# google/sbsim

Measured on AMD Instinct MI355X. Metric: zone-updates/sec (env-steps/sec x 9 zones) at batch=64k buildings per GPU, higher is better.
Workload: dtype f64

## Files before the change

### sbsim_amd/csrc/sb_device.h

```cpp
#ifndef SBSIM_AMD_SB_DEVICE_H_
#define SBSIM_AMD_SB_DEVICE_H_

#include <hip/hip_runtime.h>

#include <stdint.h>

#include "sb_layout.h"
#include "sbsim_amd.h"

namespace sb {

constexpr double kCAir = 1006.0;
constexpr double kCWater = 4180.0;
constexpr double kRhoWater = 1000.0;
constexpr double kGravity = 9.8;
constexpr int kNScal = 20;
constexpr double kAgeNone = -1e300;
__host__ __device__ inline bool age_is_none(double age) { return age < -1e200; }
constexpr int kModeMask = 0xff, kValveBit = 0x100;

struct Dev {
  int B, H, W, Z, N, Np, ncls, pitch, NL;
  int S, nsteps;
  unsigned S_magic;
  int nbands, fast;
  int ts;
  int lds_wave_doubles;
  int off_agtab, off_zscr, off_zmode;
  const uint8_t *cls;
  const double *ctab;
  const int *czone;
  const int *zone_off;
  const int *zone_cells_l;
  const uint4 *zl16;
  const int *zblk_zone;
  int n_zblocks;
  const int4 *sched;
  const unsigned long long *smask;
  int reg;
  int NR;
  int P;
  int T;
  int state_doubles;
  const uint8_t *tcls;
  const uint8_t *tcset;
  const double *tmulS;
  int tmul_doubles;
  const double *csetab;
  int ncset;
  int csetab_doubles;
  int two_sym, two_level;
  double *two_abuf;
  const int *zs_off;
  int tail_set_base, tail_pad_set;
  int RS;
  int AS;
  int ZRS;
  int Ws;
  int stream_ms;
  int n_ring;
  double n_ring_f64;
  int lw[4], l0[2], rowbase[2], nch[2];
  int lag;
  int nslots;
  float pred_haste;
  float pred_slack;
  int two_skip;
  float skip_kappa;
  int pred_first;
  int lds_reg_bytes;
  int wg_per_cu;
  int r_seam, r_A, r_zscr, r_xchg, r_zoff, r_zmode;
  int r_cmap;
  const unsigned long long *cmapS;
  const unsigned long long *amapS;
  const unsigned long long *zmapS;
  const int *cell_state;
  double *ring;
  double *temp;
  double *zmean;
  double *zair;
  double *damper;
  double *qz;
  int *mode;
  double *scal;
  struct Bld *bld;
  double *gtabg;
  double *zsum;
  double *gsum;
  int *nsw;
  int *next_b;
  int sweep_wgs;
  int *redo_ctr;
  int *redo_list;
  double *redo_scratch;
  int redo_mode;
  int roll_exact;
  int dbg_redo_mod;
  int roll_free;
  int O, col_ahu, col_blr, col_aux;
  const int *col_zone;
  const double *obs_mean, *obs_sigma;
  int n_src, n_hist, hist_normalize;
  const int *src_dest, *hist_col, *hist_off;
  const double *hist_bins;
  const int *act_kind, *act_zone;
  const double *act_lo, *act_hi;
  const int *zone_act;
  int n_damper_actions;
  long long *dbg;
  int dbg_timeline;
  sb_params p;
  const double *bp;
  const double *ctab_b;
  int off_wtab;
};

__host__ __device__ __forceinline__ double param_field(const sb_params &p, int k) {
  switch (k) {
    case SB_BP_VAV_MAX_AIR_FLOW: return p.vav_max_air_flow;
    case SB_BP_VAV_MAX_WATER_FLOW: return p.vav_max_water_flow;
    case SB_BP_AHU_RECIRC: return p.ahu_recirc;
    case SB_BP_AHU_HEAT_SP: return p.ahu_heat_sp;
    case SB_BP_AHU_COOL_SP: return p.ahu_cool_sp;
    case SB_BP_AHU_DP: return p.ahu_dp;
    case SB_BP_AHU_EFF: return p.ahu_eff;
    case SB_BP_AHU_MAX_FLOW: return p.ahu_max_flow;
    case SB_BP_BLR_SETPOINT: return p.blr_setpoint;
    case SB_BP_BLR_HEAD: return p.blr_head;
    case SB_BP_BLR_PUMP_EFF: return p.blr_pump_eff;
    case SB_BP_BLR_HEATING_RATE: return p.blr_heating_rate;
    case SB_BP_BLR_COOLING_RATE: return p.blr_cooling_rate;
    case SB_BP_BLR_CONV: return p.blr_conv;
    case SB_BP_BLR_LEN: return p.blr_len;
    case SB_BP_BLR_RADIUS: return p.blr_radius;
    case SB_BP_BLR_CAPACITY: return p.blr_capacity;
    case SB_BP_BLR_INS_K: return p.blr_ins_k;
    case SB_BP_BLR_INS_THICK: return p.blr_ins_thick;
    case SB_BP_COMFORT_LO: return p.comfort_lo;
    case SB_BP_COMFORT_HI: return p.comfort_hi;
    case SB_BP_ECO_LO: return p.eco_lo;
    case SB_BP_ECO_HI: return p.eco_hi;
    case SB_BP_MAX_PROD: return p.max_prod;
    case SB_BP_MIN_PROD: return p.min_prod;
    case SB_BP_MAX_ELEC: return p.max_elec;
    case SB_BP_MAX_GAS: return p.max_gas;
    case SB_BP_PROD_DELTA: return p.prod_delta;
    case SB_BP_PROD_STIFF: return p.prod_stiff;
    case SB_BP_W_PROD: return p.w_prod;
    case SB_BP_W_COST: return p.w_cost;
    default: return p.w_carbon;
  }
}

__device__ __forceinline__ double bparam(const Dev &a, int k, int b) {
  return a.bp ? a.bp[(size_t)k * a.B + b] : param_field(a.p, k);
}

struct ClockView {
  const double *rows;
  const int *offs;
  int pos, prev, n_rows;
  int own_prev;
};

template <bool CLK>
__device__ __forceinline__ int clock_row(const ClockView &c, int b) {
  if constexpr (CLK) return c.offs[b] + c.pos;
  else return 0;
}
template <bool CLK>
__device__ __forceinline__ double clocked(const ClockView &c, int row, int field, double scalar) {
  if constexpr (CLK) return c.rows[(size_t)row * SB_CLOCK_FIELDS + field];
  else return scalar;
}

struct StepArgs {
  const float *actions;
  float *obs, *reward, *info;
  sb_step_in in;
  ClockView clk;
};

int launch_sweep_lds(const Dev &d, int workgroups, int waves_per_wg, size_t lds_bytes, hipStream_t stream);
int prepare_sweep_lds(const Dev &d, size_t lds_bytes);
int launch_sweep_reg(const Dev &d, int cus, hipStream_t stream);
int prepare_sweep_reg(const Dev &d);
int launch_sweep_roll(const Dev &d, hipStream_t stream);
int prepare_sweep_roll(const Dev &d);
int launch_sweep_two(const Dev &d, hipStream_t stream);
int prepare_sweep_two(const Dev &d);
int launch_sweep_band(const Dev &d, hipStream_t stream);
int prepare_sweep_band(const Dev &d);
int launch_sweep_stream(const Dev &d, double *abuf, int waves, hipStream_t stream);
int prepare_sweep_stream(const Dev &d, int waves);
int launch_sweep_stream_ms(const Dev &d, double *abuf, double *ebuf, int waves, hipStream_t stream);
int prepare_sweep_stream_ms(const Dev &d, int waves);

template <int CTRL, int ROW_MASK>
__device__ __forceinline__ double dpp_or_zero(double x) {
  const int lo = __builtin_amdgcn_update_dpp(0, __double2loint(x), CTRL, ROW_MASK, 0xf, true);
  const int hi = __builtin_amdgcn_update_dpp(0, __double2hiint(x), CTRL, ROW_MASK, 0xf, true);
  return __hiloint2double(hi, lo);
}
__device__ __forceinline__ double wave_sum(double v) {
  double t = v + dpp_or_zero<0x111, 0xf>(v);
  t += dpp_or_zero<0x112, 0xf>(v);
  t += dpp_or_zero<0x113, 0xf>(v);
  t += dpp_or_zero<0x114, 0xf>(t);
  t += dpp_or_zero<0x118, 0xf>(t);
  t += dpp_or_zero<0x142, 0xa>(t);
  t += dpp_or_zero<0x143, 0xc>(t);
  const int lo = __builtin_amdgcn_readlane(__double2loint(t), 63);
  const int hi = __builtin_amdgcn_readlane(__double2hiint(t), 63);
  return __hiloint2double(hi, lo);
}
__device__ __forceinline__ double wave_max(double v) {
  double t = fmax(v, dpp_or_zero<0x111, 0xf>(v));
  t = fmax(t, dpp_or_zero<0x112, 0xf>(v));
  t = fmax(t, dpp_or_zero<0x113, 0xf>(v));
  t = fmax(t, dpp_or_zero<0x114, 0xf>(t));
  t = fmax(t, dpp_or_zero<0x118, 0xf>(t));
  t = fmax(t, dpp_or_zero<0x142, 0xa>(t));
  t = fmax(t, dpp_or_zero<0x143, 0xc>(t));
  const int lo = __builtin_amdgcn_readlane(__double2loint(t), 63);
  const int hi = __builtin_amdgcn_readlane(__double2hiint(t), 63);
  return __hiloint2double(hi, lo);
}
__device__ __forceinline__ int wave_max_i32(int v) {
  int t = max(v, __builtin_amdgcn_update_dpp(0, v, 0x111, 0xf, 0xf, true));
  t = max(t, __builtin_amdgcn_update_dpp(0, v, 0x112, 0xf, 0xf, true));
  t = max(t, __builtin_amdgcn_update_dpp(0, v, 0x113, 0xf, 0xf, true));
  t = max(t, __builtin_amdgcn_update_dpp(0, t, 0x114, 0xf, 0xf, true));
  t = max(t, __builtin_amdgcn_update_dpp(0, t, 0x118, 0xf, 0xf, true));
  t = max(t, __builtin_amdgcn_update_dpp(t, t, 0x142, 0xa, 0xf, false));
  t = max(t, __builtin_amdgcn_update_dpp(t, t, 0x143, 0xc, 0xf, false));
  return __builtin_amdgcn_readlane(t, 63);
}
__device__ __forceinline__ double wave_min(double v) {
#pragma unroll
  for (int o = 32; o > 0; o >>= 1) v = fmin(v, __shfl_xor(v, o, 64));
  return v;
}

__device__ __forceinline__ double ahu_supply(double mixed, double heat_sp, double cool_sp) {
  if (mixed > cool_sp) return cool_sp;
  if (mixed < heat_sp) return heat_sp;
  return mixed;
}

__device__ __forceinline__ int default_control(int mode, double tz, double hsp, double csp) {
// ... 451 lines not shown
```

### sbsim_amd/csrc/sbsim_hip.hip

```cpp
#include <hip/hip_runtime.h>

#include <algorithm>
#include <cmath>
#include <cstdlib>
#include <cstring>
#include <memory>
#include <string>
#include <vector>

#include "sb_host.h"
#include "step_two_cfg.h"

#ifndef SB_EXPERIMENTAL
namespace sb {
int launch_sweep_stream_ms(const Dev &, double *, double *, int, hipStream_t) { return (int)hipErrorNotSupported; }
int prepare_sweep_stream_ms(const Dev &, int) { return (int)hipErrorNotSupported; }
}
#endif

using namespace sb;

namespace {

struct Knobs {
  PlanKnobs plan;
  bool force_jacobi_global = env_flag("SBSIM_FORCE_JACOBI_GLOBAL");
  int jacobi_global_wgs = std::max(0, env_int("SBSIM_DEBUG_JACOBI_GLOBAL_WGS", 0));
  bool two_no_skip = env_flag("SBSIM_TWO_NO_SKIP");
  float pred_haste = (float)env_double("SBSIM_DEBUG_PRED_HASTE", 1.0);
  float pred_slack = (float)env_double("SBSIM_DEBUG_PRED_SLACK", 1.0);
  int pred_first = getenv("SBSIM_DEBUG_PRED_FIRST") ? std::max(1, env_int("SBSIM_DEBUG_PRED_FIRST", 1)) : 0;
  float skip_kappa = (float)std::min(100.0, std::max(0.0, env_double("SBSIM_DEBUG_SKIP_KAPPA", 0.9)));
  bool roll_exact = env_int("SBSIM_ROLL_EXACT", 0) != 0;
  int force_redo = std::max(0, env_int("SBSIM_DEBUG_FORCE_REDO", 0));
  bool roll_free = env_int("SBSIM_ROLL_FREE", 1) != 0;
  bool force_generic = env_flag("SBSIM_FORCE_GENERIC_SWEEP");
  bool phase_timing = getenv("SBSIM_PHASE_TIMING") != nullptr;
  bool debug_timeline = getenv("SBSIM_DEBUG_TIMELINE") != nullptr;
};

struct ActionTable {
  std::vector<int> zone_act;
  int n_damper_actions = 0;
};

int check_create_args(const sb_plan_desc *plan, const sb_params *params, const sb_obs_layout *obs, int n_buildings,
                      ActionTable &acts) {
  int rc = check_plan(plan);
  if (rc != SB_OK) return rc;
  if (n_buildings < 1) return fail(SB_ERR_INVALID, "sb_create: n_buildings must be >= 1");
  if (params->dt <= 0 || params->iter_limit < 1)
    return fail(SB_ERR_INVALID, "sb_create: time_step_sec and iteration_limit must be positive");
  if (params->ahu_cool_sp <= params->ahu_heat_sp)
    return fail(SB_ERR_INVALID, "cooling_air_temp_setpoint must greater than heating_air_temp_setpoint");
  if (params->n_actions < 1 || params->n_actions > 3 + plan->Z)
    return fail(SB_ERR_INVALID, "sb_create: n_actions must be in 1 .. 3 + zones (one column per settable field)");
  if (!params->act_kind || !params->act_zone || !params->act_lo || !params->act_hi)
    return fail(SB_ERR_INVALID, "sb_create: null action table (sb_params.act_kind / act_zone / act_lo / act_hi)");
  acts.zone_act.assign((size_t)std::max(plan->Z, 1), -1);
  int seen[3] = {0, 0, 0};
  for (int i = 0; i < params->n_actions; ++i) {
    const int kind = params->act_kind[i];
    if (kind < SB_ACT_BOILER_SUPPLY_WATER_SETPOINT || kind > SB_ACT_VAV_SUPPLY_AIR_DAMPER_COMMAND)
      return fail(SB_ERR_INVALID, "sb_create: unknown action kind");
    if (kind == SB_ACT_VAV_SUPPLY_AIR_DAMPER_COMMAND) {
      const int z = params->act_zone[i];
      if (z < 0 || z >= plan->Z) return fail(SB_ERR_INVALID, "sb_create: VAV action for a zone the floor plan does not have");
      if (acts.zone_act[z] >= 0) return fail(SB_ERR_INVALID, "sb_create: two action columns drive the same VAV damper");
      acts.zone_act[z] = i;
      ++acts.n_damper_actions;
    } else if (seen[kind]++) {
      return fail(SB_ERR_INVALID, "sb_create: two action columns drive the same setpoint");
    }
  }
  if (obs->n_obs < 1) return fail(SB_ERR_INVALID, "sb_create: empty observation layout");
  if (!obs->mean || !obs->sigma || (plan->Z > 0 && !obs->col_zone))
    return fail(SB_ERR_INVALID, "sb_create: null observation-layout table");
  {
    const int n_fields = obs->n_src ? obs->n_src : obs->n_obs, n_ahu = params->ahu_has_weather ? 9 : 8;
    bool ok = obs->col_ahu >= 0 && obs->col_ahu + n_ahu <= n_fields && obs->col_boiler >= 0 &&
              obs->col_boiler + 3 <= n_fields && obs->col_aux >= 0 && obs->col_aux + SB_NUM_AUX <= obs->n_obs;
    for (int z = 0; z < plan->Z; ++z) ok = ok && obs->col_zone[z] >= 0 && obs->col_zone[z] + 3 <= n_fields;
    if (!ok) return fail(SB_ERR_INVALID, "sb_create: observation columns outside the observation row");
  }
  for (int z = 0; z < plan->Z; ++z)
    if (plan->zone_off[z + 1] == plan->zone_off[z]) return fail(SB_ERR_INVALID, "sb_create: a zone without cells");
  if (obs->n_src) {
    const int n_dev_fields = 3 * plan->Z + (params->ahu_has_weather ? 9 : 8) + 3;
    if (obs->n_src != n_dev_fields || !obs->src_dest || obs->n_hist < 0 ||
        (obs->n_hist > 0 && (!obs->hist_col || !obs->hist_off || !obs->hist_bins)))
      return fail(SB_ERR_INVALID, "sb_create: inconsistent histogram-reducer layout");
    for (int i = 0; i < obs->n_src; ++i)
      if (obs->src_dest[i] >= obs->n_obs || obs->src_dest[i] < -obs->n_hist)
        return fail(SB_ERR_INVALID, "sb_create: histogram-reducer destination out of range");
    for (int j = 0; j < obs->n_hist; ++j) {
      const int n = obs->hist_off[j + 1] - obs->hist_off[j];
      if (n < 1 || obs->hist_col[j] < 0 || obs->hist_col[j] + n > obs->n_obs)
        return fail(SB_ERR_INVALID, "sb_create: histogram columns out of range");
    }
  }
  return SB_OK;
}

int setup_reg(sb_handle *h, const sb_plan_desc *plan, const RegPlan &r, const Knobs &k) {
  Dev &d = h->d;
  for (int g = 0; g < d.N; ++g) h->h_state_index[g] = r.cell_state[g];
  d.pitch = d.W; d.NL = d.N; d.ts = r.ts;
  d.NR = r.NR; d.RS = r.RS; d.Ws = r.Ws; d.n_ring = r.n_ring; d.n_ring_f64 = (double)r.n_ring;
  d.T = r.T; d.state_doubles = r.state_doubles; d.AS = r.AS; d.ZRS = r.ZRS ? r.ZRS : (r.RS | 1);
  for (int w = 0; w < 2; ++w) { d.l0[w] = r.l0[w]; d.rowbase[w] = r.rowbase[w]; d.nch[w] = r.nch[w]; }
  for (int w = 0; w < 4; ++w) d.lw[w] = r.lw[w];
  d.lag = r.lag; d.nslots = r.nslots; d.nsteps = r.steps;
  d.lds_reg_bytes = r.lds_bytes; d.wg_per_cu = r.wg_per_cu;
  d.r_seam = r.r_seam; d.r_A = r.r_A; d.r_xchg = r.r_xchg;
  if (h->kernel == SB_KERNEL_ROLL) { d.r_cmap = r.r_cmap; d.lds_wave_doubles = r.wave_doubles; }
  d.pred_haste = k.pred_haste; d.pred_slack = k.pred_slack;
  if (h->kernel == SB_KERNEL_TWO_ROWS && !k.two_no_skip) {
    bool mono = true;
    for (int c = 0; c < plan->n_classes; ++c) {
      double sum = 0.0;
      for (int j = 0; j < 4; ++j) { mono = mono && plan->class_coef[c * 8 + j] >= 0.0; sum += plan->class_coef[c * 8 + j]; }
      mono = mono && sum <= 1.0;
    }
    d.two_skip = mono ? 1 : 0;
  }
  d.skip_kappa = k.skip_kappa;
  d.pred_first = h->kernel == SB_KERNEL_BAND ? 2 : 3;
  if (k.pred_first) d.pred_first = k.pred_first;
  SB_CHECK(upload(h->zone_cells_l, plan->zone_cells, (size_t)plan->zone_off[plan->Z]));
  SB_CHECK(upload(h->cmapS, r.cmapS.data(), r.cmapS.size()));
  SB_CHECK(upload(h->amapS, r.amapS.data(), r.amapS.size()));
  SB_CHECK(upload(h->zmapS, r.zmapS.data(), r.zmapS.size()));
  SB_CHECK(upload(h->cell_state, r.cell_state.data(), r.cell_state.size()));
  SB_CHECK(alloc_zero(h->ring, (size_t)d.B * std::max(r.n_ring, 1)));
  SB_CHECK(upload(h->tcls, r.tcls.data(), r.tcls.size()));
  SB_CHECK(upload(h->tcset, r.tcset.data(), r.tcset.size()));
  SB_CHECK(upload(h->csetab, r.csetab.data(), r.csetab.size()));
  SB_CHECK(upload(h->tmul, r.tmul.data(), r.tmul.size()));
  d.tmulS = h->tmul.p; d.tmul_doubles = (int)r.tmul.size();
  d.tcset = h->tcset.p; d.csetab = h->csetab.p; d.ncset = (int)r.csetab.size() / 4;
  d.csetab_doubles = (int)r.csetab.size();
  d.two_sym = r.two_sym; d.two_level = r.two_level; d.tail_set_base = r.tail_set_base;
  d.tail_pad_set = h->kernel == SB_KERNEL_TWO_ROWS ? r.tail_pad_set : (d.ncset - 1) * 32;
  if (!r.zs_off.empty()) {
    SB_CHECK(upload(h->zs_off, r.zs_off.data(), r.zs_off.size()));
    d.zs_off = h->zs_off.p;
  }
  SB_CHECK(alloc_zero(h->temp, (size_t)d.B * d.state_doubles));
  if (h->kernel == SB_KERNEL_STREAM) {
    SB_CHECK(alloc_zero(h->abuf, (size_t)h->info.workgroups * d.state_doubles));
    if (h->stream_variant != kStreamPlain) SB_CHECK(alloc_zero(h->ebuf, (size_t)h->info.workgroups * d.state_doubles));
  }
  if (h->kernel == SB_KERNEL_TWO_ROWS) {
    SB_CHECK(alloc_zero(h->abuf, (size_t)h->info.workgroups * (size_t)std::max(1, d.NR - two::lds_slots(d.NR, d.two_level)) * 128));
    d.two_abuf = h->abuf.p;
  }
  if (h->kernel == SB_KERNEL_ROLL) {
    SB_CHECK(alloc_zero(h->redo_ctr, 2));
    SB_CHECK(alloc_zero(h->redo_list, (size_t)d.B));
    SB_CHECK(alloc_zero(h->redo_scratch, (size_t)h->info.workgroups * h->info.waves_per_workgroup * d.state_doubles));
    d.redo_ctr = h->redo_ctr.p; d.redo_list = h->redo_list.p; d.redo_scratch = h->redo_scratch.p;
    d.roll_exact = k.roll_exact; d.dbg_redo_mod = k.force_redo; d.roll_free = k.roll_free;
  }
  d.tcls = h->tcls.p;
  d.cmapS = h->cmapS.p; d.amapS = h->amapS.p; d.zmapS = h->zmapS.p; d.cell_state = h->cell_state.p;
  d.ring = h->ring.p;
  return SB_OK;
}

int setup_lds(sb_handle *h, const sb_plan_desc *plan, const LdsPlan &q, const Knobs &k) {
  Dev &d = h->d;
  for (int g = 0; g < d.N; ++g) h->h_state_index[g] = kPad + g;
  d.pitch = q.pitch; d.NL = q.NL; d.S = q.S; d.S_magic = q.S_magic; d.nsteps = q.nsteps;
  d.nbands = q.nbands; d.fast = q.fast; d.ts = q.ts;
  if (k.force_generic) d.fast = 0;
  d.off_agtab = q.off_agtab; d.off_zscr = q.off_zscr; d.off_zmode = q.off_zmode; d.off_wtab = q.off_wtab;
  d.lds_wave_doubles = q.lds_wave_doubles;
  std::vector<int> zl((size_t)plan->zone_off[plan->Z]);
  for (size_t i = 0; i < zl.size(); ++i) {
    const int g = plan->zone_cells[i];
    zl[i] = (g / d.W) * d.pitch + g % d.W;
  }
  {
    std::vector<uint8_t> padded((size_t)d.N + 2 * kPad + 8, 0);
    std::memcpy(padded.data() + kPad, plan->cell_class, (size_t)d.N);
    SB_CHECK(upload(h->cls, padded.data(), padded.size()));
  }
  SB_CHECK(upload(h->zone_cells_l, zl.data(), zl.size()));
  {
    std::vector<uint16_t> idx;
    std::vector<int> bz;
    for (int z = 0; z < d.Z; ++z) {
      const int c0 = plan->zone_off[z], c1 = plan->zone_off[z + 1];
      std::vector<uint16_t> cells;
      for (int i = c0; i < c1; ++i) cells.push_back((uint16_t)zl[i]);
      while (cells.size() % 512) cells.push_back((uint16_t)d.NL);
      for (size_t b0 = 0; b0 < cells.size(); b0 += 512) {
        for (int l = 0; l < 64; ++l)
          for (int t = 0; t < 8; ++t) idx.push_back(cells[b0 + (size_t)t * 64 + l]);
        bz.push_back(z);
      }
    }
    if (idx.empty()) { idx.assign(512, (uint16_t)d.NL); bz.push_back(0); }
    d.n_zblocks = (int)bz.size();
    SB_CHECK(upload(h->zl16, (const uint4 *)idx.data(), idx.size() / 8));
    SB_CHECK(upload(h->zblk_zone, bz.data(), bz.size()));
  }
  {
    const int nch = (d.nsteps + kChunk - 1) / kChunk;
    const int nct = ((nch + 1) & ~1) + 6;
    std::vector<int4> sc((size_t)nct * 64);
    std::vector<unsigned long long> mk((size_t)nct * kChunk, 0ull);
    for (int ch = 0; ch < nct; ++ch)
      for (int lane = 0; lane < 64; ++lane) {
        const int v0 = ch * kChunk - lane, vl = v0 + kChunk - 1;
        const int band = vl >= 0 ? vl / d.S : 0;
        const int y0 = v0 - band * d.S;
        const int rr = band * 64 + lane;
        const bool row_ok = vl >= 0 && rr < d.H;
        const int ra = std::min(rr, d.H - 1);
        const int y0a = std::min(std::max(vl >= 0 ? y0 : v0, -kChunk), d.W);
        int4 e;
        e.x = ra * d.pitch + y0a;
        e.y = ra * d.W + y0a;
        e.z = std::min(ra + 1, d.H - 1) * d.pitch + y0a;
        e.w = std::max(ra - 1, 0) * d.pitch + y0a;
        sc[(size_t)ch * 64 + lane] = e;
        for (int k = 0; k < kChunk; ++k)
          if (row_ok && y0 + k >= 0 && y0 + k < d.W) mk[(size_t)ch * kChunk + k] |= 1ull << lane;
      }
    SB_CHECK(upload(h->sched, sc.data(), sc.size()));
    SB_CHECK(upload(h->smask, mk.data(), mk.size()));
  }
  SB_CHECK(alloc_zero(h->temp, (size_t)d.B * d.Np));
  d.cls = h->cls.p; d.zl16 = h->zl16.p; d.zblk_zone = h->zblk_zone.p; d.sched = h->sched.p;
  d.smask = h->smask.p;
  return SB_OK;
}

int setup_obs_tables(sb_handle *h, const sb_params *params, const sb_obs_layout *obs, const ActionTable &acts) {
  Dev &d = h->d;
  SB_CHECK(upload(h->act_kind, params->act_kind, (size_t)params->n_actions));
  SB_CHECK(upload(h->act_zone, params->act_zone, (size_t)params->n_actions));
  SB_CHECK(upload(h->act_lo, params->act_lo, (size_t)params->n_actions));
  SB_CHECK(upload(h->act_hi, params->act_hi, (size_t)params->n_actions));
  SB_CHECK(upload(h->zone_act, acts.zone_act.data(), acts.zone_act.size()));
  d.act_kind = h->act_kind.p; d.act_zone = h->act_zone.p; d.act_lo = h->act_lo.p; d.act_hi = h->act_hi.p;
  d.zone_act = h->zone_act.p; d.n_damper_actions = acts.n_damper_actions;
  SB_CHECK(upload(h->col_zone, obs->col_zone, (size_t)d.Z));
  const size_t n_norm = (size_t)std::max(obs->n_obs, obs->n_src);
  SB_CHECK(upload(h->obs_mean, obs->mean, n_norm));
  SB_CHECK(upload(h->obs_sigma, obs->sigma, n_norm));
  d.O = obs->n_obs; d.col_ahu = obs->col_ahu; d.col_blr = obs->col_boiler; d.col_aux = obs->col_aux;
  d.col_zone = h->col_zone.p; d.obs_mean = h->obs_mean.p; d.obs_sigma = h->obs_sigma.p;
  d.n_src = obs->n_src; d.n_hist = obs->n_src ? obs->n_hist : 0; d.hist_normalize = obs->hist_normalize;
  if (obs->n_src) {
    SB_CHECK(upload(h->src_dest, obs->src_dest, (size_t)obs->n_src));
    SB_CHECK(upload(h->hist_col, obs->hist_col, (size_t)obs->n_hist));
    SB_CHECK(upload(h->hist_off, obs->hist_off, (size_t)obs->n_hist + 1));
    SB_CHECK(upload(h->hist_bins, obs->hist_bins, (size_t)(obs->n_hist ? obs->hist_off[obs->n_hist] : 0)));
    d.src_dest = h->src_dest.p; d.hist_col = h->hist_col.p; d.hist_off = h->hist_off.p;
    d.hist_bins = h->hist_bins.p;
  }
  return SB_OK;
}

int setup_state(sb_handle *h, const sb_plan_desc *plan) {
  Dev &d = h->d;
  {
    std::vector<double> ct((size_t)(d.ncls + 1) * 8, 0.0);
    std::memcpy(ct.data(), plan->class_coef, (size_t)d.ncls * 8 * sizeof(double));
    ct[(size_t)d.ncls * 8 + 4] = 1.0;
    SB_CHECK(upload(h->ctab, ct.data(), ct.size()));
  }
  SB_CHECK(upload(h->czone, plan->class_zone, (size_t)d.ncls));
  SB_CHECK(upload(h->zone_off, plan->zone_off, (size_t)d.Z + 1));
  h->h_zone_off.assign(plan->zone_off, plan->zone_off + d.Z + 1);
  h->h_zone_cells.assign(plan->zone_cells, plan->zone_cells + plan->zone_off[plan->Z]);
  SB_CHECK(alloc_zero(h->zmean, (size_t)d.B * d.Z));
  SB_CHECK(alloc_zero(h->zair, (size_t)d.B * d.Z));
  SB_CHECK(alloc_zero(h->damper, (size_t)d.B * d.Z));
  SB_CHECK(alloc_zero(h->qz, (size_t)d.B * d.Z));
  SB_CHECK(alloc_zero(h->mode, (size_t)d.B * d.Z));
  SB_CHECK(alloc_zero(h->scal, (size_t)d.B * kNScal));
  SB_CHECK(alloc_zero(h->bld, (size_t)d.B));
  SB_CHECK(alloc_zero(h->gtabg, (size_t)d.B * d.ts));
  SB_CHECK(alloc_zero(h->zsum, (size_t)d.B * d.Z));
  SB_CHECK(alloc_zero(h->gsum, (size_t)d.B));
  SB_CHECK(alloc_zero(h->nsw, (size_t)d.B));
  SB_CHECK(alloc_zero(h->next_b, 1));
  d.next_b = h->next_b.p;
  d.sweep_wgs = (d.reg && h->kernel != SB_KERNEL_ROLL) ? h->info.workgroups : h->info.workgroups * h->info.waves_per_workgroup;
  d.bld = h->bld.p; d.gtabg = h->gtabg.p; d.zsum = h->zsum.p; d.gsum = h->gsum.p; d.nsw = h->nsw.p;
  d.ctab = h->ctab.p; d.czone = h->czone.p; d.zone_off = h->zone_off.p;
  d.zone_cells_l = h->zone_cells_l.p; d.temp = h->temp.p; d.zmean = h->zmean.p;
  d.zair = h->zair.p; d.damper = h->damper.p; d.qz = h->qz.p; d.mode = h->mode.p;
  d.scal = h->scal.p;
  return SB_OK;
}

void setup_debug(sb_handle *h, const Knobs &k) {
  if (!k.phase_timing) return;
  h->d.dbg_timeline = k.debug_timeline ? 1 : 0;
  if (alloc_zero(h->dbg, 16 + (h->d.dbg_timeline ? 2048 : 0)) == SB_OK) h->d.dbg = h->dbg.p;
}

int prepare_and_reset(sb_handle *h) {
  const int e = prepare_sweep(h);
  if (e != (int)hipSuccess)
    return fail(SB_ERR_HIP, std::string("hipFuncSetAttribute(MaxDynamicSharedMemorySize): ") +
                                hipGetErrorString((hipError_t)e));
  SB_CHECK(sb_reset(h, 0.0, nullptr, nullptr));
  if (hipStreamSynchronize(nullptr) != hipSuccess) return fail(SB_ERR_HIP, "sb_create: the initial reset failed");
  return SB_OK;
}
// ... 224 lines not shown
```

### sbsim_amd/csrc/step_roll.hip

```cpp
#include "step_roll_cfg.h"
#include "sweep_common.h"

namespace sb {
namespace {

using namespace sweep;
using namespace roll;

#ifndef SB_ONE_WAIT
#define SB_ONE_WAIT 1
#endif
constexpr int kWin = 63;
constexpr int kTS = 32;
constexpr int kSeamPad = 8;

struct PairBuf {
  d2 ud0, lr0, ud1, lr1;
  d2 A;
  d2 sm;
};

struct Acc {
  double cur;
  double neg;
// ... 114 lines not shown
    e[r] = nv;
    const double sd = __hiloint2double((__double2hiint(d) & 0x7fffffff) | acc.sg, __double2loint(d));
    acc.cur = fmax(acc.cur, sd);
    acc.neg = fmin(acc.neg, sd);
    if constexpr (J + 1 < kWin)
      acc.sg = __builtin_amdgcn_update_dpp(acc.sg, acc.sg, 0x138, 0xf, 0xf, false);
    asm volatile("" : "+v"(acc.cur), "+v"(acc.neg));
  }
}

template <int NR, int S, bool EXACT>
__device__ __forceinline__ void step_ramp(double (&e)[NR], d2 ud, d2 lr, double A, Acc &acc, bool started) {
  static_assert(S < kWin, "ramp-up steps only");
  constexpr int r = S % NR, rm = (S + NR - 1) % NR, rp = (S + 1) % NR;
  const double Dn = wave_shift1<0x130, false>(e[rp], 0.0);
  double t = fma(ud.y, Dn, A);
  t = fma(lr.y, e[rp], t);
  const double U = wave_shift1<0x13c, false>(e[rm], 0.0);
  t = fma(lr.x, e[rm], t);
  const double nv = fma(ud.x, U, t);
  const double sel = started ? nv : e[r];
  if constexpr (EXACT) {
    acc.cur = fmax(acc.cur, fabs(sel - e[r]));
  } else {
#ifndef SB_EXP_NOTRACK
    asm("v_max_f32_dpp %0, %0, |%1| wave_shr:1 row_mask:0xf bank_mask:0xf bound_ctrl:1" : "+v"(acc.tr) : "v"(__double2hiint(sel - e[r])));
#endif
  }
  e[r] = sel;
}

constexpr int kA0 = 8;
template <int NR, int NAR>
struct APass {
  const unsigned long long (&cw)[(NR + 7) / 8];
  unsigned tbase;
  double *Aw, *Ax;
  double (&Areg)[NAR];
  template <int J>
  __device__ __forceinline__ d2 fetch() const {
    static_assert(kTS * 8 == 256, "a class byte (class * 8) is the byte offset into ap[] and into g[]");
    const unsigned h = (J & 7) < 4 ? (unsigned)cw[J >> 3] : (unsigned)(cw[J >> 3] >> 32);
    unsigned ad;
    if constexpr ((J & 3) == 0) asm("v_add_u32_sdwa %0, %1, %2 dst_sel:DWORD dst_unused:UNUSED_PAD src0_sel:DWORD src1_sel:BYTE_0" : "=v"(ad) : "s"(tbase), "v"(h));
    else if constexpr ((J & 3) == 1) asm("v_add_u32_sdwa %0, %1, %2 dst_sel:DWORD dst_unused:UNUSED_PAD src0_sel:DWORD src1_sel:BYTE_1" : "=v"(ad) : "s"(tbase), "v"(h));
    else if constexpr ((J & 3) == 2) asm("v_add_u32_sdwa %0, %1, %2 dst_sel:DWORD dst_unused:UNUSED_PAD src0_sel:DWORD src1_sel:BYTE_2" : "=v"(ad) : "s"(tbase), "v"(h));
    else asm("v_add_u32_sdwa %0, %1, %2 dst_sel:DWORD dst_unused:UNUSED_PAD src0_sel:DWORD src1_sel:BYTE_3" : "=v"(ad) : "s"(tbase), "v"(h));
    const __attribute__((address_space(3))) double *tp = (const __attribute__((address_space(3))) double *)ad;
    return d2{tp[0], tp[kTS]};
  }
  template <int J>
  __device__ __forceinline__ void put(const d2 &pg, const double &ej) const {
    constexpr int q = (J + 1) % NR, NL = lds_slots(NR), AS = a_stride(NR);
    double av;
    asm("v_fma_f64 %0, %1, %2, %3" : "=v"(av) : "v"(pg.x), "v"(ej), "v"(pg.y));
    if constexpr (q < AS) Aw[q] = av;
    else if constexpr (q < NL) Ax[q - AS] = av;
    else Areg[q - NL] = av;
  }
};

#ifndef SB_DEPTH
#define SB_DEPTH 1
#endif
constexpr int kDepth = SB_DEPTH;
constexpr int kBufs = kDepth + 1;
constexpr int pair_buf(int S) { return ((S - 1) / 2) % kBufs; }

struct APrev {
  d2 v[3];
};

template <int NR, int S, int S1, bool WRAP, bool EXACT, bool APASS, bool FREE, int NAR>
__device__ __forceinline__ void roll_pairs(double (&e)[NR], double (&bk)[kWin], double (&Areg)[NAR],
                                           PairBuf (&pb)[kBufs], Ctx<NR> &x, Acc &acc, const APass<NR, NAR> &ap,
                                           const APrev pv = APrev{}) {
  if constexpr (S < S1) {
    static_assert(!APASS || S1 <= kWin, "the A pass belongs to the ramp-up");
    constexpr bool wrapped = WRAP && S + 2 * kDepth >= S1;
    constexpr int N = wrapped ? S + 2 * kDepth - NR : S + 2 * kDepth;
    PairBuf &cur = pb[pair_buf(S)], &nxt = pb[pair_buf(N)];
#if SB_ONE_WAIT
    if constexpr (S < kWin) asm volatile("" ::"v"(cur.ud0.x), "v"(cur.A.x), "v"(cur.ud1.x), "v"(cur.lr1.x));
    else asm volatile("" ::"v"(cur.ud0.x), "v"(cur.A.x), "v"(cur.sm.x), "v"(cur.ud1.x), "v"(cur.lr1.x));
    __builtin_amdgcn_sched_barrier(0);
#endif
    load_first<NR, N, !wrapped>(nxt, x, Areg);
    constexpr int j0 = kA0 + 3 * ((S - 1) / 2), jp = j0 - 3;
    static_assert(!APASS || (S % 2 == 1 && jp >= S + 2 * kDepth + 2), "a slot's A is written before the pair that reads it ahead");
    static_assert(!APASS || jp >= S + 2, "a slot still holds Tprev when its A is formed");
    static_assert(!APASS || S + 2 < S1 || j0 >= NR, "the ramp-up's last pair asks for no slot: no pair would form its A");
    if constexpr (APASS && S > 1) {
      if constexpr (jp < NR) ap.template put<jp < NR ? jp : 0>(pv.v[0], e[jp < NR ? jp : 0]);
      if constexpr (jp + 1 < NR) ap.template put<jp + 1 < NR ? jp + 1 : 0>(pv.v[1], e[jp + 1 < NR ? jp + 1 : 0]);
      if constexpr (jp + 2 < NR) ap.template put<jp + 2 < NR ? jp + 2 : 0>(pv.v[2], e[jp + 2 < NR ? jp + 2 : 0]);
    }
    bool m0 = false, m1 = false;
    if constexpr (S < kWin) m0 = lanes_upto<S < kWin ? S : 0>();
    if constexpr (S + 1 < kWin) m1 = lanes_upto<S + 1 < kWin ? S + 1 : 0>();
    APrev pa{{d2{0.0, 0.0}, d2{0.0, 0.0}, d2{0.0, 0.0}}};
    if constexpr (APASS && j0 < NR) pa.v[0] = ap.template fetch<j0 < NR ? j0 : 0>();
    if constexpr (APASS && j0 + 1 < NR) pa.v[1] = ap.template fetch<j0 + 1 < NR ? j0 + 1 : 0>();
    if constexpr (APASS && j0 + 2 < NR) pa.v[2] = ap.template fetch<j0 + 2 < NR ? j0 + 2 : 0>();
    __builtin_amdgcn_sched_barrier(0);
    if constexpr (S < kWin) step_ramp<NR, S, EXACT>(e, cur.ud0, cur.lr0, cur.A.x, acc, m0);
    else step<NR, S, EXACT, FREE>(e, bk, cur.ud0, cur.lr0, cur.A.x, cur.sm.x, acc);
    __builtin_amdgcn_sched_barrier(0);
    load_second<NR, N + 1>(nxt, x);
    __builtin_amdgcn_sched_barrier(0);
    if constexpr (S + 1 < kWin) step_ramp<NR, S + 1, EXACT>(e, cur.ud1, cur.lr1, cur.A.y, acc, m1);
    else step<NR, S + 1, EXACT, FREE>(e, bk, cur.ud1, cur.lr1, cur.A.y, cur.sm.y, acc);
    __builtin_amdgcn_sched_barrier(0);
    roll_pairs<NR, S + 2, S1, WRAP, EXACT, APASS, FREE>(e, bk, Areg, pb, x, acc, ap, pa);
  }
}

template <int NR, int J>
__device__ __forceinline__ void hand_over(double (&e)[NR], const double (&bk)[kWin], const unsigned long long (&zw)[NR / 8],
                                          double *tp, const double *np_, double *zrow) {
  static_assert(NR % 8 == 0, "whole zone words");
  if constexpr (J < NR) {
    if constexpr (J < kWin) e[J] = lanes_upto<J>() ? bk[J] : e[J];
    if constexpr (J + 1 < kWin) e[J + 1] = lanes_upto<J + 1>() ? bk[J + 1] : e[J + 1];
    const unsigned w = (J & 7) < 4 ? (unsigned)zw[J / 8] : (unsigned)(zw[J / 8] >> 32);
    const unsigned off0 = (w >> (8 * (J & 3))) & 0xffu, off1 = (w >> (8 * ((J + 1) & 3))) & 0xffu;
#ifndef SB_EXP_NOMEM
    __builtin_nontemporal_store(d2{e[J], e[J + 1]}, (d2 *)(tp + J * 64));
#endif
    __hip_atomic_fetch_add((double *)((char *)zrow + off0), e[J], __ATOMIC_RELAXED, __HIP_MEMORY_SCOPE_WORKGROUP);
    __hip_atomic_fetch_add((double *)((char *)zrow + off1), e[J + 1], __ATOMIC_RELAXED, __HIP_MEMORY_SCOPE_WORKGROUP);
#ifndef SB_EXP_NOMEM
    const d2 nv = __builtin_nontemporal_load((const d2 *)(np_ + J * 64));
    e[J] = nv.x;
    e[J + 1] = nv.y;
#endif
    if constexpr ((J & 7) == 6) __builtin_amdgcn_sched_barrier(0);
    hand_over<NR, J + 2>(e, bk, zw, tp, np_, zrow);
  }
}

template <int NR>
__device__ __forceinline__ void row63_to_tail(const double (&e)[NR], Acc &acc, int lane, double &U0, double &U1) {
  constexpr int last = (NR + kWin - 1) % NR;
  const double ul = wave_shift1<0x13c, false>(e[last], 0.0);
  double &sr = (NR - 1) % 2 == 0 ? acc.sre : acc.sro;
  sr = wave_shift1<0x138, true>(sr, ul);
  const int rev = (63 - lane) * 4;
  U0 = __hiloint2double(__builtin_amdgcn_ds_bpermute(rev, __double2hiint(acc.sre)),
                        __builtin_amdgcn_ds_bpermute(rev, __double2loint(acc.sre)));
  U1 = __hiloint2double(__builtin_amdgcn_ds_bpermute(rev, __double2hiint(acc.sro)),
                        __builtin_amdgcn_ds_bpermute(rev, __double2loint(acc.sro)));
}

extern __shared__ __attribute__((aligned(16))) double lds[];

template <int NR, bool EXACT>
__global__ void __launch_bounds__(64 * kWaves) __attribute__((amdgpu_waves_per_eu(1, 1))) k_sweep_roll(Dev a) {
  const int nB = a.redo_mode ? __builtin_amdgcn_readfirstlane(a.redo_ctr[0]) : a.B;
  if (nB == 0) return;
  const int lane = threadIdx.x & 63;
  const int wave = __builtin_amdgcn_readfirstlane((int)threadIdx.x >> 6);
  const int gw = (int)blockIdx.x * kWaves + wave;
  constexpr int kASlots = (NR + 7) / 8, kZSlots = NR / 8, kCW = NR / 8;
  static_assert((NR / 2) % kBufs == 0, "pair buffers rotate through a whole period: pair_buf() must not alias across the wrap");
  constexpr int kNL = lds_slots(NR), kAS = a_stride(NR), kNAR = NR - kNL > 0 ? NR - kNL : 2;

  double *tabc = lds;
  unsigned long long *ctab8 = (unsigned long long *)(lds + a.r_cmap);
  double *tmul = lds + a.r_cmap + kCW * 64;
  double *wl = tmul + a.tmul_doubles + (size_t)wave * a.lds_wave_doubles;
  double *tapg = wl;
  double *tE0 = wl + a.r_seam + 2;
  double *A = wl + a.r_A;
  for (int i = threadIdx.x; i < a.lds_reg_bytes / 8; i += blockDim.x) lds[i] = 0.0;
  __syncthreads();
  for (int i = threadIdx.x; i < 4 * kTS; i += blockDim.x) tabc[i] = i < 4 * a.ncset ? a.csetab[i] : 0.0;
  for (int i = threadIdx.x; i < kCW * 64; i += blockDim.x) ctab8[i] = a.cmapS[i];
  for (int i = threadIdx.x; i < a.tmul_doubles; i += blockDim.x) tmul[i] = a.tmulS[i];
  if (lane < kTS) tapg[lane] = lane <= a.ncls ? a.ctab[lane * 8 + 4] : 0.0;
  __syncthreads();

  const sb_params &p = a.p;
  const int R = lane;
  constexpr int RS = 64;
  if ((unsigned)(size_t)(__attribute__((address_space(3))) double *)tabc != 0u) __builtin_trap();
  Ctx<NR> x;
  x.Arow = A + (size_t)R * kAS;
  x.Aext = A + 64 * kAS + (size_t)R * (kNL - kAS);
  x.seam = tE0 - kWin;
  x.cw = ctab8 + lane;
  x.w = x.wn = 0;
#ifdef SB_EXP_NOCOEF
  x.kc = d2{0.2 + 1e-9 * opaque(lane), 0.2};
#endif
  const bool tactive = tail_col<NR>(lane, 0) >= 0;
  const int tc0 = tactive ? tail_col<NR>(lane, 0) : 0;
  const int tcw = tactive ? tc0 : -2;
  int tset[kTailMax], tcls8[kTailMax];
#pragma unroll
  for (int t = 0; t < kTailMax; ++t) {
    tset[t] = (a.ncset - 1) * 32 * 0x10001;
    tcls8[t] = (8 * a.ncls) | ((8 * a.ncls) << 8);
    if (t < a.T && tactive) {
      const int c0 = tc0, c1 = tc0 + 1;
      tset[t] = ((int)a.tcset[t * NR + c0] << 2) | ((int)a.tcset[t * NR + c1] << 18);
      tcls8[t] = (int)a.tcls[t * NR + c0] | ((int)a.tcls[t * NR + c1] << 8);
    }
  }
  const unsigned long long *amap = a.amapS + lane;
  const unsigned long long *zmap = a.zmapS + lane;

#ifdef SB_PHASE_STAMPS
#define SB_STAMP(i) do { if (a.dbg && gw == 0 && iter == 10 && lane == 0) a.dbg[i] = (long long)__builtin_readcyclecounter(); } while (0)
#else
#define SB_STAMP(i) do { } while (0)
#endif

  double e[NR];
  double nx_g = 0.0, nx_tail[kTailMax][2] = {{0.0, 0.0}, {0.0, 0.0}}, nx_tnow = 0.0, nx_lo = 0.0, nx_hi = 0.0;
#define SB_LOAD_AUX(bb)                                                                         \
  do {                                                                                          \
    nx_tnow = a.bld[(bb)].t_now;                                                                \
    nx_lo = a.scal[(size_t)(bb) * kNScal + 16];                                                 \
    nx_hi = a.scal[(size_t)(bb) * kNScal + 17];                                                 \
    nx_g = a.gtabg[(size_t)(bb) * kTS + (opaque(lane) & (kTS - 1))];  \
    const double *tt_ = a.temp + (size_t)(bb) * a.state_doubles + NR * 64;                      \
    _Pragma("unroll") for (int t = 0; t < kTailMax; ++t)                                        \
      _Pragma("unroll") for (int k = 0; k < 2; ++k)                                             \
        if (t < a.T) nx_tail[t][k] = tt_[t * NR + tc0 + k];                                     \
  } while (0)
  auto building = [&](int s) { return a.redo_mode ? __builtin_amdgcn_readfirstlane(a.redo_list[s]) : s; };
  const int b_first = gw < nB ? building(gw) : 0;
  if (gw < nB) {
    const double *tp_ = a.temp + (size_t)b_first * a.state_doubles;
#pragma unroll
    for (int j = 0; j < NR; j += 2) {
      const d2 v = __builtin_nontemporal_load((const d2 *)(tp_ + j * 64 + 2 * R));
      e[j] = v.x;
      e[j + 1] = v.y;
    }
    SB_LOAD_AUX(b_first);
  }
  unsigned long long amapw[kASlots];
#define SB_LOAD_AMAP(g0, g1)                                                                    \
  do {                                                                                          \
    const int o_ = opaque(0);                                                                   \
    _Pragma("unroll") for (int g = (g0); g < (g1); ++g) amapw[g] = amap[o_ + g * 64];           \
  } while (0)
  constexpr int kAHalf = kASlots / 2;
  SB_LOAD_AMAP(0, kASlots);
  int iter = 0;
  for (int s = gw, sn = 0, b = b_first, bn = 0; s < nB; s = sn, b = bn, ++iter) {
    int nb = 0;
    if (lane == 0) nb = atomicAdd(a.next_b, 1);
    SB_STAMP(0);
    x.wn = x.cw[0];
    __builtin_amdgcn_sched_barrier(0);
    const double t_now = nx_tnow;
    const double ring_d = a.n_ring > 0 ? fmax(fabs(t_now - nx_lo), fabs(t_now - nx_hi)) : 0.0;
    if (lane < kTS) tapg[kTS + opaque(lane)] = nx_g;
    double tv[kTailMax][2];
#pragma unroll
    for (int t = 0; t < kTailMax; ++t)
#pragma unroll
      for (int k = 0; k < 2; ++k) tv[t][k] = tactive ? nx_tail[t][k] : 0.0;
    *(d2 *)(tE0 + opaque(tcw)) = d2{tv[0][0], tv[0][1]};
    __builtin_amdgcn_wave_barrier();
    __builtin_amdgcn_sched_barrier(0);
    SB_STAMP(1);
    double At[kTailMax][2] = {{0.0, 0.0}, {0.0, 0.0}};
    if constexpr (!EXACT) {
      const double *pg[kTailMax][2];
#pragma unroll
      for (int t = 0; t < kTailMax; ++t)
#pragma unroll
        for (int k = 0; k < 2; ++k) pg[t][k] = (const double *)((const char *)tapg + ((opaque(tcls8[t]) >> (8 * k)) & 0xff));
      double tap[kTailMax][2], tg[kTailMax][2];
#pragma unroll
      for (int t = 0; t < kTailMax; ++t)
#pragma unroll
        for (int k = 0; k < 2; ++k) { tap[t][k] = pg[t][k][0]; tg[t][k] = pg[t][k][kTS]; }
#pragma unroll
      for (int t = 0; t < kTailMax; ++t)
#pragma unroll
        for (int k = 0; k < 2; ++k) At[t][k] = fma(tap[t][k], tv[t][k], tg[t][k]);
    } else {
#pragma unroll
      for (int t = 0; t < kTailMax; ++t)
#pragma unroll
        for (int k = 0; k < 2; ++k)
          if (t < a.T && tactive) {
            const int c8 = (opaque(tcls8[t]) >> (8 * k)) & 0xff;
            const double *pg = (const double *)((const char *)tapg + c8);
            At[t][k] = fma(pg[0], tv[t][k], pg[kTS]);
          }
    }

    double Areg[kNAR];
    Areg[0] = 0.0;
    const APass<NR, kNAR> ap{amapw, (unsigned)(size_t)(__attribute__((address_space(3))) double *)tapg, A + (size_t)R * kAS,
                             A + 64 * kAS + (size_t)R * (kNL - kAS), Areg};
    {
      static_assert(kA0 == 8 && kA0 + 3 * ((kWin - 3) / 2) >= NR, "the ramp-up's pairs but the last one reach the last slot");
      const d2 g0 = ap.template fetch<0>(), g1 = ap.template fetch<1>(), g2 = ap.template fetch<2>(), g3 = ap.template fetch<3>(),
               g4 = ap.template fetch<4>(), g5 = ap.template fetch<5>(), g6 = ap.template fetch<6>(), g7 = ap.template fetch<7>();
      __builtin_amdgcn_sched_barrier(0);
      ap.template put<0>(g0, e[0]); ap.template put<1>(g1, e[1]); ap.template put<2>(g2, e[2]); ap.template put<3>(g3, e[3]);
      ap.template put<4>(g4, e[4]); ap.template put<5>(g5, e[5]); ap.template put<6>(g6, e[6]); ap.template put<7>(g7, e[7]);
    }
    __builtin_amdgcn_wave_barrier();
    __builtin_amdgcn_sched_barrier(0);
    SB_STAMP(2);

    int n_sweeps = 0, converged = 0, redo = 0;
    double bk[kWin];
    {
      PairBuf pb[kBufs];
      Acc acc;
      acc.cur = 0.0; acc.neg = 0.0; acc.sg = lane == 0 ? (int)0x80000000 : 0;
      acc.tr = acc.fin = 0;
      acc.sre = acc.sro = 0.0;
      {
        const lds_d2 ct = step_set<NR, 0>(x);
        const d2 ud = ct[0], lr = ct[1];
        load_first<NR, 1, true>(pb[pair_buf(1)], x, Areg);
        load_second<NR, 2>(pb[pair_buf(1)], x);
        if constexpr (kDepth > 1) {
          load_first<NR, 3, true>(pb[pair_buf(3)], x, Areg);
          load_second<NR, 4>(pb[pair_buf(3)], x);
        }
        static_assert(kDepth <= 2, "initial fill of the pair buffers");
        step_ramp<NR, 0, EXACT>(e, ud, lr, x.Arow[1], acc, lanes_upto<0>());
      }
      __builtin_amdgcn_sched_barrier(0);
      roll_pairs<NR, 1, kWin, false, EXACT, true, false>(e, bk, Areg, pb, x, acc, ap);
#ifndef SB_STAMP_NEXT
      SB_STAMP(15);
#endif
#pragma nounroll
      for (;;) {
        __builtin_amdgcn_sched_barrier(0);
#ifdef SB_PHASE_STAMPS
#ifndef SB_STAMP_SWEEP
#define SB_STAMP_SWEEP 1
#endif
#define SB_STAMP2(i) do { if (a.dbg && gw == 0 && iter == 10 && sweep_idx == SB_STAMP_SWEEP && lane == 0) a.dbg[i] = (long long)__builtin_readcyclecounter(); } while (0)
        const int sweep_idx = n_sweeps;
#ifdef SB_STAMP_NEXT
        if (a.dbg && gw == 0 && iter == 10 && sweep_idx == SB_STAMP_SWEEP + 1 && lane == 0) a.dbg[15] = (long long)__builtin_readcyclecounter();
#endif
#else
#define SB_STAMP2(i) do { } while (0)
#endif
        if constexpr (!EXACT) {
          if (a.roll_free) {
            const int thr_top = __double2hiint(p.conv_threshold);
            int top = wave_max_i32(acc.tr);
            if (n_sweeps == 0) top = max(top, __double2hiint(ring_d));
#pragma nounroll
            while (top > thr_top && n_sweeps + 1 < p.iter_limit) {
              __builtin_amdgcn_sched_barrier(0);
              roll_pairs<NR, kWin, NR + kWin, true, false, false, true>(e, bk, Areg, pb, x, acc, ap);
              double F0, F1;
              row63_to_tail<NR>(e, acc, lane, F0, F1);
              tail_pass_static_values<NR>(a.T, tmul + opaque(tc0), tE0 + opaque(tcw), F0, F1, tv, tset, At);
              pb[pair_buf(kWin)].sm = *(const d2 *)(x.seam + kWin);
              if constexpr (kDepth > 1) pb[pair_buf(kWin + 2)].sm = *(const d2 *)(x.seam + kWin + 2);
              ++n_sweeps;
              acc.fin = 0;
              acc.tr = lanes_upto<62>() ? acc.tr : 0;
              top = wave_max_i32(acc.tr);
              __builtin_amdgcn_sched_barrier(0);
            }
          }
        }
        SB_STAMP2(10);
        roll_pairs<NR, kWin, NR + kWin, true, EXACT, false, false>(e, bk, Areg, pb, x, acc, ap);
        SB_STAMP2(11);
        double U0, U1;
        row63_to_tail<NR>(e, acc, lane, U0, U1);
        SB_STAMP2(12);
        const double dt_ = tail_pass_static<NR>(a.T, tmul + opaque(tc0), tE0 + opaque(tcw), U0, U1, tv, tset, At);

        SB_STAMP2(13);
        if constexpr (EXACT) {
          double md = wave_max(fmax(acc.cur, dt_));
          if (n_sweeps == 0) md = fmax(md, ring_d);
          ++n_sweeps;
          converged = md <= p.conv_threshold;
        } else {
          asm("v_max_f32 %0, %0, %1" : "+v"(acc.fin) : "v"(acc.tr));
          int m_hi = max(__builtin_amdgcn_readlane(acc.fin, 63), wave_max_i32(__double2hiint(dt_)));
          if (n_sweeps == 0) m_hi = max(m_hi, __double2hiint(ring_d));
          const int thr_hi = __double2hiint(p.conv_threshold);
          ++n_sweeps;
          acc.fin = 0;
          acc.tr = lanes_upto<62>() ? acc.tr : 0;
          const bool undecided = m_hi == thr_hi || (a.dbg_redo_mod > 0 && b % a.dbg_redo_mod == 0);
          if (m_hi <= thr_hi && undecided) { redo = 1; break; }
          converged = m_hi < thr_hi;
        }
        SB_STAMP2(14);
#ifdef SB_EXP_DESYNC
        if (n_sweeps >= 1 + (int)(((unsigned)b * 2654435761u >> 13) % 9u)) break;
#else
        if (converged || n_sweeps >= p.iter_limit) break;
#endif
        pb[pair_buf(kWin)].sm = *(const d2 *)(x.seam + kWin);
        if constexpr (kDepth > 1) pb[pair_buf(kWin + 2)].sm = *(const d2 *)(x.seam + kWin + 2);
        acc.cur = -acc.neg;
        acc.neg = 0.0;
        acc.sg = lane == 0 ? (int)0x80000000 : 0;
      }
    }
    __builtin_amdgcn_sched_barrier(0);
    SB_STAMP(3);
    sn = a.sweep_wgs + __builtin_amdgcn_readfirstlane(nb);
    bn = sn < nB ? building(sn) : 0;
    if (sn < nB) SB_LOAD_AUX(bn);
    SB_LOAD_AMAP(0, kAHalf);
    __builtin_amdgcn_sched_barrier(0);
    SB_STAMP(4);

    double *zs = A;
    const int ZRS = a.ZRS;
    {
      unsigned long long zw[kZSlots];
      const unsigned long long *zm = zmap + opaque(0);
#pragma unroll
      for (int g = 0; g < kZSlots; ++g) zw[g] = zm[g * 64];
      __builtin_amdgcn_sched_barrier(0);
      double *tp = redo ? a.redo_scratch + (size_t)gw * a.state_doubles : a.temp + (size_t)b * a.state_doubles;
      double *Ttail = tp + NR * 64;
      double *zrow = zs + (size_t)opaque(R) * ZRS;
      for (int z = 0; z <= a.Z; ++z) zrow[z] = 0.0;
      __builtin_amdgcn_wave_barrier();
#pragma unroll
      for (int t = 0; t < kTailMax; ++t)
        if (t < a.T && tactive) {
          *(d2 *)(Ttail + t * NR + tc0) = d2{tv[t][0], tv[t][1]};
          zrow[a.Z] += tv[t][0] + tv[t][1];
        }
      const double *np_ = a.temp + (size_t)(sn < nB ? bn : b) * a.state_doubles;
      static_assert(RS == 64, "hand_over: slot stride");
      hand_over<NR, 0>(e, bk, zw, tp + 2 * R, np_ + 2 * R, zrow);
    }
    __builtin_amdgcn_sched_barrier(0);
    SB_STAMP(5);
    SB_LOAD_AMAP(kAHalf, kASlots);
    __builtin_amdgcn_sched_barrier(0);
    SB_STAMP(6);
    __builtin_amdgcn_wave_barrier();
    SB_STAMP(7);

    {
      double gacc = 0.0;
      for (int zb = 0; zb <= a.Z; zb += 16) {
        const int zz = zb + (lane >> 2), g = lane & 3;
        const double *zr = zs + (size_t)g * ZRS + (zz <= a.Z ? zz : a.Z);
        double part[RS / 4];
#pragma unroll
        for (int k = 0; k < RS / 4; ++k) part[k] = zr[(size_t)4 * k * ZRS];
        double v = 0.0;
#pragma unroll
        for (int k = 0; k < RS / 4; ++k) v += part[k];
        if (zz > a.Z) v = 0.0;
        v += dpp_or_zero<0xB1, 0xf>(v);
        v += dpp_or_zero<0x4E, 0xf>(v);
        if (g == 0 && zz < a.Z && !redo) a.zsum[(size_t)b * a.Z + zz] = v;
        if (g == 0 && zz <= a.Z) gacc += v;
      }
      const double gsum = wave_sum(gacc);
      if (lane == 0 && !redo) {
        a.gsum[b] = gsum + a.n_ring_f64 * t_now;
        a.nsw[b] = n_sweeps | (converged << 16);
      }
      if (lane == 0 && redo) a.redo_list[atomicAdd(a.redo_ctr, 1)] = b;
      SB_STAMP(8);
#ifdef SB_PHASE_STAMPS
      if (a.dbg && gw == 0 && iter == 10 && lane == 0) a.dbg[9] = n_sweeps;
#endif
    }
  }
#undef SB_STAMP
#undef SB_LOAD_AUX
#undef SB_LOAD_AMAP
}

}

int sweep_roll_redo_workgroups() { return 8; }

namespace {

template <int NR>
int prepare(const Dev &d) {
  const int e = (int)hipFuncSetAttribute((const void *)k_sweep_roll<NR, false>, hipFuncAttributeMaxDynamicSharedMemorySize,
                                         d.lds_reg_bytes);
  if (e != (int)hipSuccess) return e;
  return (int)hipFuncSetAttribute((const void *)k_sweep_roll<NR, true>, hipFuncAttributeMaxDynamicSharedMemorySize,
                                  d.lds_reg_bytes);
}

template <int NR>
int launch(const Dev &d, hipStream_t stream) {
  const dim3 grid((d.sweep_wgs + kWaves - 1) / kWaves), block(64 * kWaves);
  if (d.roll_exact) {
    hipLaunchKernelGGL((k_sweep_roll<NR, true>), grid, block, (size_t)d.lds_reg_bytes, stream, d);
    return (int)hipGetLastError();
  }
  hipLaunchKernelGGL((k_sweep_roll<NR, false>), grid, block, (size_t)d.lds_reg_bytes, stream, d);
  Dev r = d;
  r.redo_mode = 1;
  r.next_b = d.redo_ctr + 1;
  r.sweep_wgs = sweep_roll_redo_workgroups() * kWaves;
  hipLaunchKernelGGL((k_sweep_roll<NR, true>), dim3(sweep_roll_redo_workgroups()), block, (size_t)d.lds_reg_bytes, stream, r);
  return (int)hipGetLastError();
}

}

int prepare_sweep_roll(const Dev &d) {
  if (d.NR == 96) return prepare<96>(d);
  if (d.NR == 88) return prepare<88>(d);
  if (d.NR == 80) return prepare<80>(d);
  if (d.NR == 72) return prepare<72>(d);
  if (d.NR == 64) return prepare<64>(d);
  return (int)hipErrorInvalidValue;
}

int launch_sweep_roll(const Dev &d, hipStream_t stream) {
  if (d.NR == 96) return launch<96>(d, stream);
  if (d.NR == 88) return launch<88>(d, stream);
  if (d.NR == 80) return launch<80>(d, stream);
  if (d.NR == 72) return launch<72>(d, stream);
  if (d.NR == 64) return launch<64>(d, stream);
  return (int)hipErrorInvalidValue;
}

}
```

Before: 308.7 million.

## Add static-then-dynamic building scheduling to roll sweep and ballot-based convergence check

Adds an optional scheme where each wave processes a fixed number of rounds of buildings in static stride order before switching to atomic work-stealing, controlled by a new env var that defaults to fully dynamic. It also replaces the wave max reduction in the roll-free convergence loop with a ballot test, which needs only a single wave instruction. The zone-map loads are hoisted ahead of the next-building computation. The ballot change and the load hoist are active by default, while the static scheduling is inert unless the env var is set.

```diff
diff --git a/sbsim_amd/csrc/sb_device.h b/sbsim_amd/csrc/sb_device.h
--- a/sbsim_amd/csrc/sb_device.h
+++ b/sbsim_amd/csrc/sb_device.h
@@ -97,6 +97,8 @@
   int redo_mode;
   int roll_exact;
   int dbg_redo_mod;
+  int roll_dynamic_rounds;
+  int roll_static;
   int roll_free;
   int O, col_ahu, col_blr, col_aux;
   const int *col_zone;
diff --git a/sbsim_amd/csrc/sbsim_hip.hip b/sbsim_amd/csrc/sbsim_hip.hip
--- a/sbsim_amd/csrc/sbsim_hip.hip
+++ b/sbsim_amd/csrc/sbsim_hip.hip
@@ -33,6 +33,7 @@
   float skip_kappa = (float)std::min(100.0, std::max(0.0, env_double("SBSIM_DEBUG_SKIP_KAPPA", 0.9)));
   bool roll_exact = env_int("SBSIM_ROLL_EXACT", 0) != 0;
   int force_redo = std::max(0, env_int("SBSIM_DEBUG_FORCE_REDO", 0));
+  int roll_dynamic_rounds = std::max(0, env_int("SBSIM_ROLL_DYNAMIC_ROUNDS", 1 << 30));
   bool roll_free = env_int("SBSIM_ROLL_FREE", 1) != 0;
   bool force_generic = env_flag("SBSIM_FORCE_GENERIC_SWEEP");
   bool phase_timing = getenv("SBSIM_PHASE_TIMING") != nullptr;
@@ -161,6 +162,7 @@
     SB_CHECK(alloc_zero(h->redo_scratch, (size_t)h->info.workgroups * h->info.waves_per_workgroup * d.state_doubles));
     d.redo_ctr = h->redo_ctr.p; d.redo_list = h->redo_list.p; d.redo_scratch = h->redo_scratch.p;
     d.roll_exact = k.roll_exact; d.dbg_redo_mod = k.force_redo; d.roll_free = k.roll_free;
+    d.roll_dynamic_rounds = k.roll_dynamic_rounds;
   }
   d.tcls = h->tcls.p;
   d.cmapS = h->cmapS.p; d.amapS = h->amapS.p; d.zmapS = h->zmapS.p; d.cell_state = h->cell_state.p;
diff --git a/sbsim_amd/csrc/step_roll.hip b/sbsim_amd/csrc/step_roll.hip
--- a/sbsim_amd/csrc/step_roll.hip
+++ b/sbsim_amd/csrc/step_roll.hip
@@ -290,6 +290,8 @@
                         __builtin_amdgcn_ds_bpermute(rev, __double2loint(acc.sro)));
 }
 
+__device__ __forceinline__ bool any_above(int w, int thr) { return __builtin_amdgcn_ballot_w64(w > thr) != 0; }
+
 extern __shared__ __attribute__((aligned(16))) double lds[];
 
 template <int NR, bool EXACT>
@@ -387,10 +389,18 @@
   } while (0)
   constexpr int kAHalf = kASlots / 2;
   SB_LOAD_AMAP(0, kASlots);
+  const int n_static = a.roll_static;
+  const int draw_base = a.sweep_wgs * (n_static > 1 ? n_static : 1);
   int iter = 0;
   for (int s = gw, sn = 0, b = b_first, bn = 0; s < nB; s = sn, b = bn, ++iter) {
+    const bool draws = iter + 1 >= n_static;
     int nb = 0;
-    if (lane == 0) nb = atomicAdd(a.next_b, 1);
+#if defined(SB_PHASE_STAMPS) && defined(SB_STAMP_DRAW)
+    SB_STAMP(15);
+#endif
+    if (draws) {
+      if (lane == 0) nb = atomicAdd(a.next_b, 1);
+    }
     SB_STAMP(0);
     x.wn = x.cw[0];
     __builtin_amdgcn_sched_barrier(0);
@@ -472,7 +482,7 @@
       }
       __builtin_amdgcn_sched_barrier(0);
       roll_pairs<NR, 1, kWin, false, EXACT, true, false>(e, bk, Areg, pb, x, acc, ap);
-#ifndef SB_STAMP_NEXT
+#if !defined(SB_STAMP_NEXT) && !defined(SB_STAMP_DRAW)
       SB_STAMP(15);
 #endif
 #pragma nounroll
@@ -493,10 +503,10 @@
         if constexpr (!EXACT) {
           if (a.roll_free) {
             const int thr_top = __double2hiint(p.conv_threshold);
-            int top = wave_max_i32(acc.tr);
-            if (n_sweeps == 0) top = max(top, __double2hiint(ring_d));
+            bool top = any_above(acc.tr, thr_top);
+            if (n_sweeps == 0) top = top || __double2hiint(ring_d) > thr_top;
 #pragma nounroll
-            while (top > thr_top && n_sweeps + 1 < p.iter_limit) {
+            while (top && n_sweeps + 1 < p.iter_limit) {
               __builtin_amdgcn_sched_barrier(0);
               roll_pairs<NR, kWin, NR + kWin, true, false, false, true>(e, bk, Areg, pb, x, acc, ap);
               double F0, F1;
@@ -507,7 +517,7 @@
               ++n_sweeps;
               acc.fin = 0;
               acc.tr = lanes_upto<62>() ? acc.tr : 0;
-              top = wave_max_i32(acc.tr);
+              top = any_above(acc.tr, thr_top);
               __builtin_amdgcn_sched_barrier(0);
             }
           }
@@ -528,9 +538,9 @@
           converged = md <= p.conv_threshold;
         } else {
           asm("v_max_f32 %0, %0, %1" : "+v"(acc.fin) : "v"(acc.tr));
+          const int thr_hi = __double2hiint(p.conv_threshold);
           int m_hi = max(__builtin_amdgcn_readlane(acc.fin, 63), wave_max_i32(__double2hiint(dt_)));
           if (n_sweeps == 0) m_hi = max(m_hi, __double2hiint(ring_d));
-          const int thr_hi = __double2hiint(p.conv_threshold);
           ++n_sweeps;
           acc.fin = 0;
           acc.tr = lanes_upto<62>() ? acc.tr : 0;
@@ -553,7 +563,14 @@
     }
     __builtin_amdgcn_sched_barrier(0);
     SB_STAMP(3);
-    sn = a.sweep_wgs + __builtin_amdgcn_readfirstlane(nb);
+    unsigned long long zw[kZSlots];
+    {
+      const unsigned long long *zm = zmap + opaque(0);
+#pragma unroll
+      for (int g = 0; g < kZSlots; ++g) zw[g] = zm[g * 64];
+    }
+    __builtin_amdgcn_sched_barrier(0);
+    sn = draws ? draw_base + __builtin_amdgcn_readfirstlane(nb) : s + a.sweep_wgs;
     bn = sn < nB ? building(sn) : 0;
     if (sn < nB) SB_LOAD_AUX(bn);
     SB_LOAD_AMAP(0, kAHalf);
@@ -563,11 +580,6 @@
     double *zs = A;
     const int ZRS = a.ZRS;
     {
-      unsigned long long zw[kZSlots];
-      const unsigned long long *zm = zmap + opaque(0);
-#pragma unroll
-      for (int g = 0; g < kZSlots; ++g) zw[g] = zm[g * 64];
-      __builtin_amdgcn_sched_barrier(0);
       double *tp = redo ? a.redo_scratch + (size_t)gw * a.state_doubles : a.temp + (size_t)b * a.state_doubles;
       double *Ttail = tp + NR * 64;
       double *zrow = zs + (size_t)opaque(R) * ZRS;
@@ -643,13 +655,17 @@
 template <int NR>
 int launch(const Dev &d, hipStream_t stream) {
   const dim3 grid((d.sweep_wgs + kWaves - 1) / kWaves), block(64 * kWaves);
+  Dev f = d;
+  const int rounds = d.sweep_wgs > 0 ? d.B / d.sweep_wgs : 0;
+  f.roll_static = rounds > d.roll_dynamic_rounds ? rounds - d.roll_dynamic_rounds : 0;
   if (d.roll_exact) {
-    hipLaunchKernelGGL((k_sweep_roll<NR, true>), grid, block, (size_t)d.lds_reg_bytes, stream, d);
+    hipLaunchKernelGGL((k_sweep_roll<NR, true>), grid, block, (size_t)d.lds_reg_bytes, stream, f);
     return (int)hipGetLastError();
   }
-  hipLaunchKernelGGL((k_sweep_roll<NR, false>), grid, block, (size_t)d.lds_reg_bytes, stream, d);
+  hipLaunchKernelGGL((k_sweep_roll<NR, false>), grid, block, (size_t)d.lds_reg_bytes, stream, f);
   Dev r = d;
   r.redo_mode = 1;
+  r.roll_static = 0;
   r.next_b = d.redo_ctr + 1;
   r.sweep_wgs = sweep_roll_redo_workgroups() * kWaves;
   hipLaunchKernelGGL((k_sweep_roll<NR, true>), dim3(sweep_roll_redo_workgroups()), block, (size_t)d.lds_reg_bytes, stream, r);
```

Measured after the change: 308.5 million, median of 3. No clear change (-0.0%).
